# Aatricks/LightDiffusion-Next

Hardware: AMD Instinct MI355X
Metric: sampler it/s (UNet steps/sec) SD1.5 1024x1024 bs=1 bf16 (higher is better)
Workload: dtype bf16

## Files before the change

### lightdiffusion-next_amd/csrc/ff_block.hip

```cpp
#include <hip/hip_runtime.h>
#include <stdint.h>
#include <stdlib.h>
#include "ldx_device.h"
#include "ldx_kernels.h"
#include "rowblock_store.h"

namespace ldx {

constexpr int FB_C = 320, FB_I = 1280, FB_BM = 128, FB_CH = 128, FB_NCH = FB_I / FB_CH;
constexpr int FB_AROW = FB_C * 2 + 16;
constexpr int FB_GROW = FB_CH * 2 + 16;
constexpr int FB_ABYTES = FB_BM * FB_AROW, FB_GBYTES = FB_BM * FB_GROW;
constexpr int FB_LDS = FB_ABYTES + 2 * FB_GBYTES + 2 * FB_C * 4;
static_assert(FB_C == RB_C && FB_BM == RB_BM && FB_AROW == RB_AROW, "rb_layernorm_rows writes this A tile");

template <typename T>
__global__ __launch_bounds__(512, 1) void ff_block_kernel(const FFBlockArgs p) {
    extern __shared__ __attribute__((aligned(16))) char smem[];
    using V8 = typename Vec<T>::v8;
    char* sA = smem;
    char* sGb = smem + FB_ABYTES;
    float* sG = (float*)(smem + FB_ABYTES + 2 * FB_GBYTES);
    float* sBt = sG + FB_C;
    const int tid = threadIdx.x, lane = tid & 63;
    const int wave = __builtin_amdgcn_readfirstlane(tid >> 6);
    const int l15 = lane & 15, g4 = lane >> 4;
    const long m0 = (long)blockIdx.x * FB_BM;
    T* __restrict__ Hp = (T*)p.H;
    const T* __restrict__ W1 = (const T*)p.W1;
    const T* __restrict__ W2 = (const T*)p.W2;

    for (int i = tid; i < FB_C; i += 512) { sG[i] = p.ln_g[i]; sBt[i] = p.ln_b[i]; }
    rb_layernorm_rows<T>(Hp, p.ldh, m0, p.M, p.eps, sG, sBt, sA, tid, false);
    __syncthreads();

    f32x4 y[3][8];
#pragma unroll
    for (int t = 0; t < 3; ++t)
#pragma unroll
        for (int qt = 0; qt < 8; ++qt) y[t][qt] = (f32x4){0.f, 0.f, 0.f, 0.f};

    constexpr int NKS = FB_C / 32, PD = 2;
    uint4 w1[PD + 1][2];
    auto w1_rows = [&](int ch, const T*& wv, const T*& wg) __attribute__((always_inline)) {
        const int i0 = ch * FB_CH + wave * 16;
        const int vrow = (i0 >> 5) * 64 + (i0 & 31) + l15;
        wv = W1 + (long)vrow * FB_C + g4 * 8;
        wg = wv + 32 * FB_C;
    };
    {
        const T *wv, *wg;
        w1_rows(0, wv, wg);
#pragma unroll
        for (int ks = 0; ks < PD; ++ks) { w1[ks][0] = *(const uint4*)(wv + ks * 32); w1[ks][1] = *(const uint4*)(wg + ks * 32); }
    }
    auto w2_load = [&](int ch, int ks, uint4 (&w2f)[4][3]) __attribute__((always_inline)) {
        const T* w2 = W2 + (long)(wave * 40) * FB_I + ch * FB_CH + g4 * 8;
#pragma unroll
        for (int t = 0; t < 3; ++t) {
            const int r = 16 * t + l15;
            w2f[ks][t] = (r < 40) ? *(const uint4*)(w2 + (long)r * FB_I + ks * 32) : make_uint4(0, 0, 0, 0);
        }
    };
    for (int ch = 0; ch < FB_NCH; ++ch) {
        char* sGc = sGb + (ch & 1) * FB_GBYTES;
        uint4 w2f[4][3];
        {
            const T *wv, *wg;
            w1_rows(ch, wv, wg);
            f32x4 tv[8], tg[8];
#pragma unroll
            for (int qt = 0; qt < 8; ++qt) { tv[qt] = (f32x4){0.f, 0.f, 0.f, 0.f}; tg[qt] = (f32x4){0.f, 0.f, 0.f, 0.f}; }
#pragma unroll
            for (int ks = 0; ks < NKS; ++ks) {
                if (ks + PD < NKS) { w1[(ks + PD) % (PD + 1)][0] = *(const uint4*)(wv + (ks + PD) * 32); w1[(ks + PD) % (PD + 1)][1] = *(const uint4*)(wg + (ks + PD) * 32); }
                V8 af[8];
#pragma unroll
                for (int qt = 0; qt < 8; ++qt) af[qt] = as_v8<T>(*(const uint4*)(sA + (16 * qt + l15) * FB_AROW + (ks * 32 + g4 * 8) * 2));
                const V8 a8 = as_v8<T>(w1[ks % (PD + 1)][0]), g8 = as_v8<T>(w1[ks % (PD + 1)][1]);
#pragma unroll
                for (int qt = 0; qt < 8; ++qt) { tv[qt] = mfma16(a8, af[qt], tv[qt]); tg[qt] = mfma16(g8, af[qt], tg[qt]); }
                __builtin_amdgcn_sched_barrier(0);
            }
            w2_load(ch, 0, w2f);
            const int i0 = ch * FB_CH + wave * 16;
            const int brow = (i0 >> 5) * 64 + (i0 & 31) + 4 * g4;
            const float4 bv = *(const float4*)(p.b1 + brow), bg = *(const float4*)(p.b1 + brow + 32);
#pragma unroll
            for (int qt = 0; qt < 8; ++qt) {
                const float v0 = (tv[qt][0] + bv.x) * gelu_erf_f(tg[qt][0] + bg.x), v1 = (tv[qt][1] + bv.y) * gelu_erf_f(tg[qt][1] + bg.y);
                const float v2 = (tv[qt][2] + bv.z) * gelu_erf_f(tg[qt][2] + bg.z), v3 = (tv[qt][3] + bv.w) * gelu_erf_f(tg[qt][3] + bg.w);
                *(uint2*)(sGc + (16 * qt + l15) * FB_GROW + (wave * 16 + 4 * g4) * 2) = pack4<T>(v0, v1, v2, v3);
            }
        }
        __syncthreads();
        w2_load(ch, 1, w2f); w2_load(ch, 2, w2f); w2_load(ch, 3, w2f);
        if (ch + 1 < FB_NCH) {
            const T *wv, *wg;
            w1_rows(ch + 1, wv, wg);
#pragma unroll
            for (int ks = 0; ks < PD; ++ks) { w1[ks][0] = *(const uint4*)(wv + ks * 32); w1[ks][1] = *(const uint4*)(wg + ks * 32); }
        }
#pragma unroll
        for (int ks = 0; ks < 4; ++ks) {
            V8 gf[8];
#pragma unroll
            for (int qt = 0; qt < 8; ++qt) gf[qt] = as_v8<T>(*(const uint4*)(sGc + (16 * qt + l15) * FB_GROW + (ks * 32 + g4 * 8) * 2));
#pragma unroll
            for (int t = 0; t < 3; ++t) {
                const V8 w8 = as_v8<T>(w2f[ks][t]);
#pragma unroll
                for (int qt = 0; qt < 8; ++qt) y[t][qt] = mfma16(w8, gf[qt], y[t][qt]);
            }
            __builtin_amdgcn_sched_barrier(0);
        }
    }

    uint2 rr[3][8];
#pragma unroll
    for (int t = 0; t < 3; ++t)
#pragma unroll
        for (int qt = 0; qt < 8; ++qt) {
            const long m = m0 + 16 * qt + l15;
            const int nl = 16 * t + 4 * g4;
            rr[t][qt] = (m < p.M && nl < 40) ? *(const uint2*)(Hp + m * p.ldh + wave * 40 + nl) : make_uint2(0u, 0u);
        }
#pragma unroll
    for (int t = 0; t < 3; ++t) {
        const int nl = 16 * t + 4 * g4;
        const int n = wave * 40 + (nl < 40 ? nl : 0);
        const float4 bo = p.b2 ? *(const float4*)(p.b2 + n) : make_float4(0.f, 0.f, 0.f, 0.f);
#pragma unroll
        for (int qt = 0; qt < 8; ++qt) {
            float r4[4];
            unpack4<T>(rr[t][qt], r4);
            rr[t][qt] = pack4<T>(y[t][qt][0] + bo.x + r4[0], y[t][qt][1] + bo.y + r4[1], y[t][qt][2] + bo.z + r4[2], y[t][qt][3] + bo.w + r4[3]);
        }
    }
    __syncthreads();
    rb_store_rows<T, 8>(Hp, p.ldh, m0, p.M, 0, wave, l15, g4, tid, rr, sGb);
}

bool ff_block_ok(const FFBlockArgs& a) {
    return g_plan_sw.ff_fuse && a.C == FB_C && a.inner == FB_I && a.M > 0 && a.ldh % 8 == 0 && a.b1 != nullptr;
}
template <typename T>
static void launch_ff_t(const FFBlockArgs& a, hipStream_t s) {
    static DevOnce once;
    set_dyn_lds(once, (const void*)ff_block_kernel<T>, FB_LDS);
    hipLaunchKernelGGL((ff_block_kernel<T>), dim3((unsigned)((a.M + FB_BM - 1) / FB_BM)), dim3(512), FB_LDS, s, a);
}
void launch_ff_block(const FFBlockArgs& a, DType dt, hipStream_t s) {
    if (dt == DT_BF16) launch_ff_t<__bf16>(a, s); else launch_ff_t<_Float16>(a, s);
}

}
```

### lightdiffusion-next_amd/csrc/rowblock_store.h

```cpp
#pragma once
#include "ldx_device.h"

namespace ldx {

constexpr int RB_SROW = 320 * 2 + 16;
constexpr int RB_STAGE_BYTES = 64 * RB_SROW;
constexpr int RB_C = 320, RB_BM = 128;
constexpr int RB_AROW = RB_C * 2 + 16;

template <typename T>
__device__ __forceinline__ void rb_layernorm_rows(const T* __restrict__ Hp, const int ldh, const long m0, const long M, const float eps, const float* sG,
                                                  const float* sBt, char* sA, const int tid, const bool no_loads) {
    const int row = tid >> 2, part = tid & 3;
    const long m = m0 + row;
    float x[80];
    if (m < M && !no_loads) {
#pragma unroll
        for (int j = 0; j < 10; ++j) {
            const uint4 u = *(const uint4*)(Hp + m * ldh + (part + 4 * j) * 8);
            float f[8];
            unpack8<T>(u, f);
#pragma unroll
            for (int e = 0; e < 8; ++e) x[8 * j + e] = f[e];
        }
    } else {
#pragma unroll
        for (int e = 0; e < 80; ++e) x[e] = 0.f;
    }
    float su = 0.f;
#pragma unroll
    for (int e = 0; e < 80; ++e) su += x[e];
    su += dpp_f<0xB1>(su); su += dpp_f<0x4E>(su);
    const float mean = su * (1.0f / RB_C);
    float sq = 0.f;
#pragma unroll
    for (int e = 0; e < 80; ++e) { const float d = x[e] - mean; sq = fmaf(d, d, sq); }
    sq += dpp_f<0xB1>(sq); sq += dpp_f<0x4E>(sq);
    const float rstd = rsqrtf(sq * (1.0f / RB_C) + eps);
    __syncthreads();
#pragma unroll
    for (int j = 0; j < 10; ++j) {
        const int c0 = (part + 4 * j) * 8;
        float f[8];
#pragma unroll
        for (int e = 0; e < 8; ++e) f[e] = fmaf((x[8 * j + e] - mean) * rstd, sG[c0 + e], sBt[c0 + e]);
        *(uint4*)(sA + row * RB_AROW + c0 * 2) = pack8<T>(f);
    }
}

template <typename T, int QT>
__device__ __forceinline__ void rb_store_rows(T* __restrict__ Y, const int ldy, const long m0, const long M, const int col0, const int wave, const int l15,
                                              const int g4, const int tid, const uint2 (&out)[3][QT], char* sS, const long dup_rows = 0) {
    int tid_ = tid, l15_ = l15;
    asm volatile("" : "+v"(tid_), "+v"(l15_));
#pragma unroll
    for (int hh = 0; hh < QT / 4; ++hh) {
#pragma unroll
        for (int t = 0; t < 3; ++t) {
            const int nl = 16 * t + 4 * g4;
            if (nl < 40) {
#pragma unroll
                for (int q4 = 0; q4 < 4; ++q4) *(uint2*)(sS + (16 * q4 + l15_) * RB_SROW + (wave * 40 + nl) * 2) = out[t][4 * hh + q4];
            }
        }
        __syncthreads();
#pragma unroll
        for (int j = 0; j < 5; ++j) {
            const int idx = tid_ + 512 * j, row = idx / 40, ch = idx - row * 40;
            const long m = m0 + 64 * hh + row;
            if (m < M) {
                const uint4 v = *(const uint4*)(sS + row * RB_SROW + ch * 16);
                *(uint4*)(Y + m * ldy + col0 + ch * 8) = v;
                if (dup_rows) *(uint4*)(Y + (m + dup_rows) * ldy + col0 + ch * 8) = v;
            }
        }
        __syncthreads();
    }
}

}
```

### lightdiffusion-next_amd/csrc/rowgemm.hip

```cpp
#include <hip/hip_runtime.h>
#include <stdint.h>
#include <stdlib.h>
#include "ldx_device.h"
#include "ldx_kernels.h"
#include "rowblock_store.h"

namespace ldx {

template <int CC> struct RgGeom {
    static constexpr int BM = 128 * 320 / CC, QT = BM / 16, LPR = 512 / BM, NH = CC / 320;
    static constexpr int AROW = CC * 2 + 16, ABYTES = BM * AROW;
    static constexpr int TAB = 2 * CC * 4 + 8 * 64 * 4 + 64 * 4;
    static constexpr int LDS = ABYTES + TAB + RB_STAGE_BYTES;
};

template <typename T, int PRO, int CC>
__global__ __launch_bounds__(512, 1) void rowgemm_kernel(const RowGemmArgs p) {
    using G = RgGeom<CC>;
    constexpr int RG_C = CC, RG_BM = G::BM, RG_AROW = G::AROW, RG_ABYTES = G::ABYTES, QT = G::QT, LPR = G::LPR;
    extern __shared__ __attribute__((aligned(16))) char smem[];
    using V8 = typename Vec<T>::v8;
    char* sA = smem;
    float* sSc = (float*)(smem + RG_ABYTES);
    float* sSh = sSc + RG_C;
    float* sRed = sSh + RG_C;
    float* sMR = sRed + 8 * 64;
    const int tid = threadIdx.x, lane = tid & 63;
    const int wave = __builtin_amdgcn_readfirstlane(tid >> 6);
    const int l15_0 = lane & 15, g4_0 = lane >> 4;
    const long m0 = (long)blockIdx.x * RG_BM;
    const T* __restrict__ Xp = (const T*)p.X;
    const T* __restrict__ W = (const T*)p.W;

    const int nown = p.N / G::NH;
    const int npass = nown / 320;
    constexpr int NKS = RG_C / 32, PD = 3;
    uint4 wf[PD + 1][3];
    auto wload = [&](int wrow0_, int l15_, int g4_, int ks, int slot) __attribute__((always_inline)) {
#pragma unroll
        for (int t = 0; t < 3; ++t) {
            const int r = 16 * t + l15_;
            wf[slot][t] = (r < 40) ? *(const uint4*)(W + (long)(wrow0_ + r) * RG_C + ks * 32 + g4_ * 8) : make_uint4(0, 0, 0, 0);
        }
    };
#pragma unroll
    for (int ks = 0; ks < PD; ++ks) wload((int)blockIdx.y * nown + wave * 40, l15_0, g4_0, ks, ks);

    if (PRO == 1) { for (int i = tid; i < RG_C; i += 512) { sSc[i] = p.g[i]; sSh[i] = p.b[i]; } }
    if (PRO == 2) {
        const int b = (int)(m0 / p.HW);
        const int g = tid & 31, st = (tid >> 5) & 1, sl = tid >> 6;
        float a = 0.f;
        {
            const float* pp = p.partial + ((long)b * p.nchunk) * p.G * 2 + g * 2 + st;
            int ck = sl;
            for (; ck + 56 < p.nchunk; ck += 64) {
                float v[8];
#pragma unroll
                for (int u = 0; u < 8; ++u) v[u] = pp[(long)(ck + 8 * u) * p.G * 2];
#pragma unroll
                for (int u = 0; u < 8; ++u) a += v[u];
            }
            for (; ck < p.nchunk; ck += 8) a += pp[(long)ck * p.G * 2];
        }
        sRed[sl * 64 + g * 2 + st] = a;
        __syncthreads();
        if (tid < 32) {
            float su = 0.f, sq = 0.f;
#pragma unroll
            for (int s8 = 0; s8 < 8; ++s8) { su += sRed[s8 * 64 + tid * 2]; sq += sRed[s8 * 64 + tid * 2 + 1]; }
            const float n = (float)p.HW * (float)(RG_C / 32);
            const float mean = su / n;
            const float var = fmaxf(sq / n - mean * mean, 0.f);
            sMR[tid] = mean; sMR[32 + tid] = rsqrtf(var + p.eps);
        }
        __syncthreads();
        for (int c = tid; c < RG_C; c += 512) {
            const int g2 = c / (RG_C / 32);
            const float a2 = sMR[32 + g2] * p.g[c];
            sSc[c] = a2; sSh[c] = p.b[c] - sMR[g2] * a2;
        }
    }
    {
        const int row = tid / LPR, part = tid % LPR;
        const long m = m0 + row;
        uint4 raw[10];
#pragma unroll
        for (int j = 0; j < 10; ++j) raw[j] = (m < p.M && !(p.abl & 4)) ? *(const uint4*)(Xp + m * p.ldx + (part + LPR * j) * 8) : make_uint4(0, 0, 0, 0);
        if (PRO == 0) {
#pragma unroll
            for (int j = 0; j < 10; ++j) *(uint4*)(sA + row * RG_AROW + (part + LPR * j) * 16) = raw[j];
        } else {
            float x[80];
#pragma unroll
            for (int j = 0; j < 10; ++j) {
                float f[8];
                unpack8<T>(raw[j], f);
#pragma unroll
                for (int e = 0; e < 8; ++e) x[8 * j + e] = f[e];
            }
            float mean = 0.f, rstd = 1.f;
            if (PRO == 1) {
                float su = 0.f;
#pragma unroll
                for (int e = 0; e < 80; ++e) su += x[e];
                su += dpp_f<0xB1>(su); su += dpp_f<0x4E>(su); if (LPR == 8) su += dpp_f<0x141>(su);
                mean = su * (1.0f / RG_C);
                float sq = 0.f;
#pragma unroll
                for (int e = 0; e < 80; ++e) { const float d = x[e] - mean; sq = fmaf(d, d, sq); }
                sq += dpp_f<0xB1>(sq); sq += dpp_f<0x4E>(sq); if (LPR == 8) sq += dpp_f<0x141>(sq);
                rstd = rsqrtf(sq * (1.0f / RG_C) + p.eps);
            }
            __syncthreads();
#pragma unroll
            for (int j = 0; j < 10; ++j) {
                const int c0 = (part + LPR * j) * 8;
                float f[8];
#pragma unroll
                for (int e = 0; e < 8; ++e)
                    f[e] = (PRO == 1) ? fmaf((x[8 * j + e] - mean) * rstd, sSc[c0 + e], sSh[c0 + e]) : fmaf(x[8 * j + e], sSc[c0 + e], sSh[c0 + e]);
                *(uint4*)(sA + row * RG_AROW + c0 * 2) = pack8<T>(f);
            }
        }
    }
    __syncthreads();

#pragma unroll 1
    for (int pass = 0; pass < npass; ++pass) {
        int l15 = l15_0, g4 = g4_0;
        asm volatile("" : "+v"(l15), "+v"(g4));
        const int wrow0 = (int)blockIdx.y * nown + pass * 320 + wave * 40;
        f32x4 acc[3][QT];
#pragma unroll
        for (int t = 0; t < 3; ++t)
#pragma unroll
            for (int qt = 0; qt < QT; ++qt) acc[t][qt] = (f32x4){0.f, 0.f, 0.f, 0.f};
        if (!(p.abl & 2))
#pragma unroll
        for (int ks = 0; ks < NKS; ++ks) {
            if (ks + PD < NKS) wload(wrow0, l15, g4, ks + PD, (ks + PD) % (PD + 1));
            V8 af[QT];
#pragma unroll
            for (int qt = 0; qt < QT; ++qt) af[qt] = as_v8<T>(*(const uint4*)(sA + (16 * qt + l15) * RG_AROW + (ks * 32 + g4 * 8) * 2));
#pragma unroll
            for (int t = 0; t < 3; ++t) {
                const V8 w8 = as_v8<T>(wf[ks % (PD + 1)][t]);
#pragma unroll
                for (int qt = 0; qt < QT; ++qt) acc[t][qt] = mfma16(w8, af[qt], acc[t][qt]);
            }
            __builtin_amdgcn_sched_barrier(0);
        }
        __builtin_amdgcn_sched_barrier(0);
        uint2 rr[3][QT];
#pragma unroll
        for (int t = 0; t < 3; ++t)
#pragma unroll
            for (int qt = 0; qt < QT; ++qt) {
                const long m = m0 + 16 * qt + l15;
                const int nl = 16 * t + 4 * g4;
                rr[t][qt] = (p.R && m < p.M && nl < 40 && !(p.abl & 1)) ? *(const uint2*)((const T*)p.R + m * p.ldr + wrow0 + nl) : make_uint2(0u, 0u);
            }
#pragma unroll
        for (int t = 0; t < 3; ++t) {
            const int nl = 16 * t + 4 * g4;
            const int n = wrow0 + (nl < 40 ? nl : 0);
            const float4 bo = p.bias ? *(const float4*)(p.bias + n) : make_float4(0.f, 0.f, 0.f, 0.f);
#pragma unroll
            for (int qt = 0; qt < QT; ++qt) {
                float r4[4];
                unpack4<T>(rr[t][qt], r4);
                rr[t][qt] = pack4<T>(acc[t][qt][0] + bo.x + r4[0], acc[t][qt][1] + bo.y + r4[1], acc[t][qt][2] + bo.z + r4[2], acc[t][qt][3] + bo.w + r4[3]);
            }
        }
        if (p.gn_out) {
            float cs[3][4], cq[3][4];
#pragma unroll
            for (int t = 0; t < 3; ++t) {
#pragma unroll
                for (int r = 0; r < 4; ++r) { cs[t][r] = 0.f; cq[t][r] = 0.f; }
#pragma unroll
                for (int qt = 0; qt < QT; ++qt) {
                    float v4[4];
                    unpack4<T>(rr[t][qt], v4);
#pragma unroll
                    for (int r = 0; r < 4; ++r) { cs[t][r] += v4[r]; cq[t][r] = fmaf(v4[r], v4[r], cq[t][r]); }
                }
#pragma unroll
                for (int r = 0; r < 4; ++r) { cs[t][r] = row16_sum(cs[t][r]); cq[t][r] = row16_sum(cq[t][r]); }
                const int nl = 16 * t + 4 * g4;
                if (l15 == 0 && nl < 40) {
#pragma unroll
                    for (int r = 0; r < 4; ++r) { sSc[(wave * 40 + nl + r) * 2] = cs[t][r]; sSc[(wave * 40 + nl + r) * 2 + 1] = cq[t][r]; }
                }
            }
            __syncthreads();
            const int cpg = p.N / 32;
            if (tid < (320 / cpg) * 2) {
                const int gl = tid >> 1, st = tid & 1;
                float a = 0.f;
                for (int c = 0; c < cpg; ++c) a += sSc[(gl * cpg + c) * 2 + st];
                const int bimg = (int)(m0 / p.HW), chunk = (int)((m0 - (long)bimg * p.HW) / RG_BM);
                const int g0 = ((int)blockIdx.y * nown + pass * 320) / cpg;
                p.gn_out[(((long)bimg * p.gn_nchunk + chunk) * 32 + g0 + gl) * 2 + st] = a;
            }
        }
        if (pass + 1 < npass) {
#pragma unroll
            for (int ks = 0; ks < PD; ++ks) wload(wrow0 + 320, l15, g4, ks, ks);
        }
        if (!(p.abl & 8)) rb_store_rows<T, QT>((T*)p.Y, p.ldy, m0, p.M, (int)blockIdx.y * nown + pass * 320, wave, l15, g4, tid, rr, smem + RG_ABYTES + G::TAB, p.dup_rows);
    }
}

bool rowgemm_ok(const RowGemmArgs& a) {
    if (!g_plan_sw.rowgemm || (a.K != 320 && a.K != 640) || (a.K == 640 && !g_plan_sw.rowgemm640) || a.N <= 0 || a.N % a.K || a.M <= 0 || a.ldx % 8 || a.ldy % 8 || (a.R && a.ldr % 4) || a.pro < 0 || a.pro > 2) return false;
    const int bm = 128 * 320 / a.K;
    if (a.pro >= 1 && (!a.g || !a.b)) return false;
    if (a.pro == 2 && (!a.partial || a.G != 32 || a.HW % bm || a.M % a.HW || a.nchunk < 1 || a.nchunk > GN_NCHUNK)) return false;
    return true;
}
template <typename T, int PRO, int CC>
static void launch_rowgemm_inst(const RowGemmArgs& a, hipStream_t s) {
    using G = RgGeom<CC>;
    static DevOnce once;
    set_dyn_lds(once, (const void*)rowgemm_kernel<T, PRO, CC>, G::LDS);
    hipLaunchKernelGGL((rowgemm_kernel<T, PRO, CC>), dim3((unsigned)((a.M + G::BM - 1) / G::BM), G::NH), dim3(512), G::LDS, s, a);
}
template <typename T>
static void launch_rowgemm_t(const RowGemmArgs& a, hipStream_t s) {
    if (a.K == 320) {
        if (a.pro == 0) launch_rowgemm_inst<T, 0, 320>(a, s); else if (a.pro == 1) launch_rowgemm_inst<T, 1, 320>(a, s); else launch_rowgemm_inst<T, 2, 320>(a, s);
    } else {
        if (a.pro == 0) launch_rowgemm_inst<T, 0, 640>(a, s); else if (a.pro == 1) launch_rowgemm_inst<T, 1, 640>(a, s); else launch_rowgemm_inst<T, 2, 640>(a, s);
    }
}
void launch_rowgemm(const RowGemmArgs& a0, DType dt, hipStream_t s) {
    static const int abl = getenv("LDX_RG_ABL") ? atoi(getenv("LDX_RG_ABL")) : 0;
    RowGemmArgs a = a0; a.abl = abl;
    if (dt == DT_BF16) launch_rowgemm_t<__bf16>(a, s); else launch_rowgemm_t<_Float16>(a, s);
}

}
```

### lightdiffusion-next_amd/csrc/xattn_block.hip

```cpp
#include <hip/hip_runtime.h>
#include <stdint.h>
#include <stdlib.h>
#include "ldx_device.h"
#include "ldx_kernels.h"
#include "rowblock_store.h"

namespace ldx {

#ifdef XA_ABLATE
__device__ int xa_dbg = 0;
#define XA_DBG(bit) (xa_dbg & (bit))
#else
#define XA_DBG(bit) false
#endif
constexpr int XA_C = 320, XA_H = 8, XA_D = 40, XA_BM = 128, XA_MK = 80;
constexpr int XA_AROW = XA_C * 2 + 16;
constexpr int XA_VROW = 96;
constexpr int XA_ABYTES = XA_BM * XA_AROW, XA_VBYTES = XA_MK * XA_VROW;
constexpr int XA_LDS = XA_ABYTES + XA_H * XA_VBYTES + 2 * XA_C * 4;
static_assert(XA_C == RB_C && XA_BM == RB_BM && XA_AROW == RB_AROW, "rb_layernorm_rows writes this A tile");

template <typename T>
__device__ __forceinline__ void xa_project(const T* __restrict__ W, const int wrow0, const char* sA, const int l15, const int g4, f32x4 (&acc)[3][8]) {
    using V8 = typename Vec<T>::v8;
    constexpr int NKS = XA_C / 32, PD = 3;
#pragma unroll
    for (int t = 0; t < 3; ++t)
#pragma unroll
        for (int qt = 0; qt < 8; ++qt) acc[t][qt] = (f32x4){0.f, 0.f, 0.f, 0.f};
    uint4 wf[PD + 1][3];
    auto wload = [&](int ks, int slot) __attribute__((always_inline)) {
#pragma unroll
        for (int t = 0; t < 3; ++t) {
            const int r = 16 * t + l15;
            uint4 u = make_uint4(0, 0, 0, 0);
            if (r < XA_D) u = *(const uint4*)(W + (long)(wrow0 + r) * XA_C + ks * 32 + g4 * 8);
            wf[slot][t] = u;
        }
    };
#pragma unroll
    for (int ks = 0; ks < PD; ++ks) wload(ks, ks);
#pragma unroll
    for (int ks = 0; ks < NKS; ++ks) {
        if (ks + PD < NKS) wload(ks + PD, (ks + PD) % (PD + 1));
        V8 af[8];
#pragma unroll
        for (int qt = 0; qt < 8; ++qt) af[qt] = as_v8<T>(*(const uint4*)(sA + (16 * qt + l15) * XA_AROW + (ks * 32 + g4 * 8) * 2));
#pragma unroll
        for (int t = 0; t < 3; ++t) {
            const V8 w8 = as_v8<T>(wf[ks % (PD + 1)][t]);
#pragma unroll
            for (int qt = 0; qt < 8; ++qt) acc[t][qt] = mfma16(w8, af[qt], acc[t][qt]);
        }
    }
}

template <typename T>
__global__ __launch_bounds__(512, 1) void xattn_block_kernel(const XAttnArgs p) {
    extern __shared__ __attribute__((aligned(16))) char smem[];
    using V8 = typename Vec<T>::v8;
    char* sA = smem;
    float* sG = (float*)(smem + XA_ABYTES + XA_H * XA_VBYTES);
    float* sBt = sG + XA_C;
    const int tid = threadIdx.x, lane = tid & 63;
    const int wave = __builtin_amdgcn_readfirstlane(tid >> 6);
    const int l15 = lane & 15, g4 = lane >> 4;
    char* sV = smem + XA_ABYTES + wave * XA_VBYTES;
    const long m0 = (long)blockIdx.x * XA_BM;
    const int b = (int)(m0 / p.N);
    T* __restrict__ Hp = (T*)p.H;

    for (int i = tid; i < XA_C; i += 512) { sG[i] = p.ln_g[i]; sBt[i] = p.ln_b[i]; }
    {
        const T* __restrict__ Vp = (const T*)p.V + (long)b * p.Mk * p.ldv + wave * XA_D;
        for (int i = lane; i < XA_VBYTES / 16; i += 64) {
            const int row = i / 6, ch = i - row * 6;
            uint4 u = make_uint4(0, 0, 0, 0);
            if (row < p.Mk && ch < 5) u = *(const uint4*)(Vp + (long)row * p.ldv + ch * 8);
            *(uint4*)(sV + row * XA_VROW + ch * 16) = u;
        }
    }
    rb_layernorm_rows<T>(Hp, p.ldh, m0, p.M, p.eps, sG, sBt, sA, tid, XA_DBG(16));
    __syncthreads();

    f32x4 qT[3][8];
    if (!XA_DBG(1)) xa_project<T>((const T*)p.Wq, wave * XA_D, sA, l15, g4, qT);
    else for (int t = 0; t < 3; ++t) for (int qt = 0; qt < 8; ++qt) qT[t][qt] = (f32x4){1.f, 1.f, 1.f, 1.f};

    V8 kf[5][2];
    {
        const T* __restrict__ Kp = (const T*)p.K + (long)b * p.Mk * p.ldk + wave * XA_D;
#pragma unroll
        for (int kt = 0; kt < 5; ++kt) {
            const int key = 16 * kt + l15;
            uint2 a0 = make_uint2(0, 0), a1 = make_uint2(0, 0), a2 = make_uint2(0, 0);
            if (key < p.Mk) {
                const T* kr = Kp + (long)key * p.ldk;
                a0 = *(const uint2*)(kr + 4 * g4);
                a1 = *(const uint2*)(kr + 16 + 4 * g4);
                if (g4 < 2) a2 = *(const uint2*)(kr + 32 + 4 * g4);
            }
            kf[kt][0] = as_v8<T>(make_uint4(a0.x, a0.y, a1.x, a1.y));
            kf[kt][1] = as_v8<T>(make_uint4(a2.x, a2.y, 0u, 0u));
        }
    }
    V8 vf[3][3];
#pragma unroll
    for (int dt = 0; dt < 3; ++dt)
#pragma unroll
        for (int j = 0; j < 3; ++j) {
            const char* vp = sV + (j * 32 + g4 * 4 + (l15 >> 2)) * XA_VROW + (dt * 16 + (l15 & 3) * 4) * 2;
            U128 u;
            u.d[0] = lds_read_tr16(vp);
            u.d[1] = (j < 2) ? lds_read_tr16(vp + 16 * XA_VROW) : make_uint2(0u, 0u);
            vf[dt][j] = as_v8<T>(u.u);
        }
    __syncthreads();

    const float c = p.scale * 1.44269504088896340736f;
#pragma unroll
    for (int qt = 0; qt < 8; ++qt) {
        if (XA_DBG(2)) break;
        V8 qb0, qb1;
#pragma unroll
        for (int e = 0; e < 4; ++e) {
            qb0[e] = (T)qT[0][qt][e]; qb0[4 + e] = (T)qT[1][qt][e];
            qb1[e] = (g4 < 2) ? (T)qT[2][qt][e] : (T)0.f; qb1[4 + e] = (T)0.f;
        }
        f32x4 s[5];
#pragma unroll
        for (int kt = 0; kt < 5; ++kt) {
            s[kt] = mfma16(kf[kt][0], qb0, (f32x4){0.f, 0.f, 0.f, 0.f});
            s[kt] = mfma16(kf[kt][1], qb1, s[kt]);
        }
        float mx = -INFINITY;
#pragma unroll
        for (int kt = 0; kt < 5; ++kt)
#pragma unroll
            for (int r = 0; r < 4; ++r) {
                if (16 * kt + 4 * g4 + r >= p.Mk) s[kt][r] = -INFINITY;
                mx = fmaxf(mx, s[kt][r]);
            }
        mx = quad_max(mx);
        const float mc = (mx == -INFINITY) ? 0.f : mx * c;
        float pv[6][4], l = 0.f;
#pragma unroll
        for (int kt = 0; kt < 5; ++kt)
#pragma unroll
            for (int r = 0; r < 4; ++r) {
                const float e = to_f32(from_f32<T>(__builtin_amdgcn_exp2f(fmaf(s[kt][r], c, -mc))));
                pv[kt][r] = e; l += e;
            }
#pragma unroll
        for (int r = 0; r < 4; ++r) pv[5][r] = 0.f;
        l = quad_sum(l);
        f32x4 o[3];
#pragma unroll
        for (int dt = 0; dt < 3; ++dt) o[dt] = (f32x4){0.f, 0.f, 0.f, 0.f};
#pragma unroll
        for (int j = 0; j < 3; ++j) {
            V8 pf;
#pragma unroll
            for (int r = 0; r < 4; ++r) { pf[r] = (T)pv[2 * j][r]; pf[4 + r] = (T)pv[2 * j + 1][r]; }
#pragma unroll
            for (int dt = 0; dt < 3; ++dt) o[dt] = mfma16(vf[dt][j], pf, o[dt]);
        }
        const float inv = (l > 0.f) ? 1.0f / l : 0.f;
        const int q = 16 * qt + l15;
#pragma unroll
        for (int dt = 0; dt < 3; ++dt) {
            const int d = 16 * dt + 4 * g4;
            if (d < XA_D) *(uint2*)(sA + q * XA_AROW + (wave * XA_D + d) * 2) = pack4<T>(o[dt][0] * inv, o[dt][1] * inv, o[dt][2] * inv, o[dt][3] * inv);
        }
    }
    __syncthreads();

    f32x4 y[3][8];
    if (!XA_DBG(4)) xa_project<T>((const T*)p.Wo, wave * XA_D, sA, l15, g4, y);
    else for (int t = 0; t < 3; ++t) for (int qt = 0; qt < 8; ++qt) y[t][qt] = (f32x4){1.f, 1.f, 1.f, 1.f};
    if (XA_DBG(8)) return;
    uint2 rr[3][8];
#pragma unroll
    for (int t = 0; t < 3; ++t)
#pragma unroll
        for (int qt = 0; qt < 8; ++qt) {
            const long m = m0 + 16 * qt + l15;
            const int nl = 16 * t + 4 * g4;
            rr[t][qt] = (m < p.M && nl < XA_D && !XA_DBG(8)) ? *(const uint2*)(Hp + m * p.ldh + wave * XA_D + nl) : make_uint2(0u, 0u);
        }
#pragma unroll
    for (int t = 0; t < 3; ++t) {
        const int nl = 16 * t + 4 * g4;
        const int n = wave * XA_D + (nl < XA_D ? nl : 0);
        const float4 bo = p.bo ? *(const float4*)(p.bo + n) : make_float4(0.f, 0.f, 0.f, 0.f);
#pragma unroll
        for (int qt = 0; qt < 8; ++qt) {
            float r4[4];
            unpack4<T>(rr[t][qt], r4);
            rr[t][qt] = pack4<T>(y[t][qt][0] + bo.x + r4[0], y[t][qt][1] + bo.y + r4[1], y[t][qt][2] + bo.z + r4[2], y[t][qt][3] + bo.w + r4[3]);
        }
    }
    rb_store_rows<T, 8>(Hp, p.ldh, m0, p.M, 0, wave, l15, g4, tid, rr, smem + XA_ABYTES);
}

bool xattn_block_ok(const XAttnArgs& a) {
    return g_plan_sw.xattn_fuse && a.C == XA_C && a.heads == XA_H && a.Mk >= 1 && a.Mk <= XA_MK && a.N % XA_BM == 0 && a.M % a.N == 0 && a.ldh % 8 == 0 && a.ldk % 4 == 0 && a.ldv % 8 == 0;
}

template <typename T>
static void launch_xattn_t(const XAttnArgs& a, hipStream_t s) {
    static DevOnce once;
    set_dyn_lds(once, (const void*)xattn_block_kernel<T>, XA_LDS);
#ifdef XA_ABLATE
    static const int dbg_once = []() { const int v = getenv("LDX_XA_DBG") ? atoi(getenv("LDX_XA_DBG")) : 0; (void)hipMemcpyToSymbol(HIP_SYMBOL(xa_dbg), &v, sizeof(int)); return v; }();
    (void)dbg_once;
#endif
    hipLaunchKernelGGL((xattn_block_kernel<T>), dim3((unsigned)((a.M + XA_BM - 1) / XA_BM)), dim3(512), XA_LDS, s, a);
}
void launch_xattn_block(const XAttnArgs& a, DType dt, hipStream_t s) {
    if (dt == DT_BF16) launch_xattn_t<__bf16>(a, s); else launch_xattn_t<_Float16>(a, s);
}

}
```

Measured before the change: 76.62.

## Swizzle LDS operand tiles instead of padding to remove bank conflicts

Replaces the +16-byte row padding of the A, G and output staging tiles in LDS with an XOR swizzle of 16-byte chunks. This covers the ff, xattn and rowblock-store paths, and rowgemm's A stride becomes +32. A constexpr bank-conflict model checks at compile time that fragment reads are conflict-free and that stores are at most 2-way. The aim is to remove the 2-way conflicts the +16 stride caused on MFMA operand reads. In exchange it adds address arithmetic and an XOR-indexed layout that every writer and reader must follow consistently.

Measured after the change: 76.55. About the same (-0.1%).

```diff
diff --git a/lightdiffusion-next_amd/csrc/ff_block.hip b/lightdiffusion-next_amd/csrc/ff_block.hip
--- a/lightdiffusion-next_amd/csrc/ff_block.hip
+++ b/lightdiffusion-next_amd/csrc/ff_block.hip
@@ -8,11 +8,16 @@
 namespace ldx {
 
 constexpr int FB_C = 320, FB_I = 1280, FB_BM = 128, FB_CH = 128, FB_NCH = FB_I / FB_CH;
-constexpr int FB_AROW = FB_C * 2 + 16;
-constexpr int FB_GROW = FB_CH * 2 + 16;
+constexpr int FB_AROW = FB_C * 2;
+constexpr int FB_GROW = FB_CH * 2;
 constexpr int FB_ABYTES = FB_BM * FB_AROW, FB_GBYTES = FB_BM * FB_GROW;
-constexpr int FB_LDS = FB_ABYTES + 2 * FB_GBYTES + 2 * FB_C * 4;
+constexpr int FB_LDS_USED = FB_ABYTES + 2 * FB_GBYTES + 2 * FB_C * 4;
+constexpr int FB_LDS = FB_BM * (FB_C * 2 + 16) + 2 * FB_BM * (FB_CH * 2 + 16) + 2 * FB_C * 4;
 static_assert(FB_C == RB_C && FB_BM == RB_BM && FB_AROW == RB_AROW, "rb_layernorm_rows writes this A tile");
+static_assert(rb_opnd_read_cycles(FB_AROW, FB_C * 2) == lds::READ_B128.floor && rb_opnd_read_cycles(FB_GROW, FB_CH * 2) == lds::READ_B128.floor,
+              "fragment reads of A and G must be conflict-free");
+static_assert(rb_opnd_colstore_cycles(FB_GROW) <= 8, "GEGLU stores: 2-way at most (the floor for 16 rows x 8 bytes)");
+static_assert(FB_LDS_USED <= FB_LDS && FB_LDS <= lds::LDS_BYTES_PER_CU && RB_STAGE_BYTES <= 2 * FB_GBYTES, "LDS budget; the output tile goes over the G buffers");
 
 template <typename T>
 __global__ __launch_bounds__(512, 1) void ff_block_kernel(const FFBlockArgs p) {
@@ -25,6 +30,8 @@
     const int tid = threadIdx.x, lane = tid & 63;
     const int wave = __builtin_amdgcn_readfirstlane(tid >> 6);
     const int l15 = lane & 15, g4 = lane >> 4;
+    const RbFragLane a_lane = rb_frag_lane(l15, g4);
+    const int g_lane = rb_opnd_ofs(l15, g4, FB_GROW);
     const long m0 = (long)blockIdx.x * FB_BM;
     T* __restrict__ Hp = (T*)p.H;
     const T* __restrict__ W1 = (const T*)p.W1;
@@ -76,7 +83,7 @@
                 if (ks + PD < NKS) { w1[(ks + PD) % (PD + 1)][0] = *(const uint4*)(wv + (ks + PD) * 32); w1[(ks + PD) % (PD + 1)][1] = *(const uint4*)(wg + (ks + PD) * 32); }
                 V8 af[8];
 #pragma unroll
-                for (int qt = 0; qt < 8; ++qt) af[qt] = as_v8<T>(*(const uint4*)(sA + (16 * qt + l15) * FB_AROW + (ks * 32 + g4 * 8) * 2));
+                for (int qt = 0; qt < 8; ++qt) af[qt] = as_v8<T>(*(const uint4*)(sA + 16 * qt * FB_AROW + ks * 64 + a_lane.base[ks & 1]));
                 const V8 a8 = as_v8<T>(w1[ks % (PD + 1)][0]), g8 = as_v8<T>(w1[ks % (PD + 1)][1]);
 #pragma unroll
                 for (int qt = 0; qt < 8; ++qt) { tv[qt] = mfma16(a8, af[qt], tv[qt]); tg[qt] = mfma16(g8, af[qt], tg[qt]); }
@@ -90,7 +97,7 @@
             for (int qt = 0; qt < 8; ++qt) {
                 const float v0 = (tv[qt][0] + bv.x) * gelu_erf_f(tg[qt][0] + bg.x), v1 = (tv[qt][1] + bv.y) * gelu_erf_f(tg[qt][1] + bg.y);
                 const float v2 = (tv[qt][2] + bv.z) * gelu_erf_f(tg[qt][2] + bg.z), v3 = (tv[qt][3] + bv.w) * gelu_erf_f(tg[qt][3] + bg.w);
-                *(uint2*)(sGc + (16 * qt + l15) * FB_GROW + (wave * 16 + 4 * g4) * 2) = pack4<T>(v0, v1, v2, v3);
+                *(uint2*)(sGc + 16 * qt * FB_GROW + rb_opnd_ofs(l15, 2 * wave + (g4 >> 1), FB_GROW) + (g4 & 1) * 8) = pack4<T>(v0, v1, v2, v3);
             }
         }
         __syncthreads();
@@ -105,7 +112,7 @@
         for (int ks = 0; ks < 4; ++ks) {
             V8 gf[8];
 #pragma unroll
-            for (int qt = 0; qt < 8; ++qt) gf[qt] = as_v8<T>(*(const uint4*)(sGc + (16 * qt + l15) * FB_GROW + (ks * 32 + g4 * 8) * 2));
+            for (int qt = 0; qt < 8; ++qt) gf[qt] = as_v8<T>(*(const uint4*)(sGc + 16 * qt * FB_GROW + (g_lane ^ (ks * 64))));
 #pragma unroll
             for (int t = 0; t < 3; ++t) {
                 const V8 w8 = as_v8<T>(w2f[ks][t]);
diff --git a/lightdiffusion-next_amd/csrc/lds_image.h b/lightdiffusion-next_amd/csrc/lds_image.h
--- /dev/null
+++ b/lightdiffusion-next_amd/csrc/lds_image.h
@@ -0,0 +1,72 @@
+#pragma once
+
+namespace ldx {
+namespace lds {
+
+struct Instr {
+    int ngroups, glanes;
+    int banks;
+    int dwords;
+    int floor;
+    int xfer;
+    bool contiguous;
+};
+
+constexpr Instr READ_B128{4, 16, 64, 4, 4, 4, false};
+constexpr Instr READ_B64{2, 32, 64, 2, 2, 2, true};
+constexpr Instr READ_B64_TR_B16{2, 32, 64, 2, 2, 2, true};
+constexpr Instr WRITE_B64{4, 16, 32, 2, 4, 6, true};
+constexpr Instr WRITE_B128{8, 8, 32, 4, 8, 13, true};
+
+constexpr int B128_GROUP_LANE[2][16] = {{0, 1, 2, 3, 12, 13, 14, 15, 20, 21, 22, 23, 24, 25, 26, 27}, {4, 5, 6, 7, 8, 9, 10, 11, 16, 17, 18, 19, 28, 29, 30, 31}};
+
+constexpr int group_lane(const Instr& in, int g, int i) {
+    return in.contiguous ? g * in.glanes + i : 32 * (g >> 1) + B128_GROUP_LANE[g & 1][i];
+}
+
+template <typename F>
+constexpr int cycles(const Instr& in, F addr) {
+    int total = 0;
+    for (int g = 0; g < in.ngroups; ++g) {
+        long seen[64][32] = {};
+        int cnt[64] = {};
+        int worst = 0;
+        for (int i = 0; i < in.glanes; ++i) {
+            const long a = addr(group_lane(in, g, i));
+            if (a < 0) continue;
+            for (int d = 0; d < in.dwords; ++d) {
+                const long dw = a / 4 + d;
+                const int b = (int)(dw % in.banks);
+                bool dup = false;
+                for (int k = 0; k < cnt[b]; ++k) dup = dup || seen[b][k] == dw + 1;
+                if (!dup) { seen[b][cnt[b]] = dw + 1; ++cnt[b]; }
+                if (cnt[b] > worst) worst = cnt[b];
+            }
+        }
+        total += worst;
+    }
+    return total;
+}
+
+template <typename F>
+constexpr int cost(const Instr& in, F addr) {
+    const int c = cycles(in, addr);
+    return c > in.xfer ? c : in.xfer;
+}
+
+constexpr int frag16_read_cycles(int stride, int base = 0) {
+    return cycles(READ_B128, [=](int lane) { return (long)base + (long)(lane & 15) * stride + (lane >> 4) * 16; });
+}
+constexpr int frag32_read_cycles(int stride, int base = 0) {
+    return cycles(READ_B128, [=](int lane) { return (long)base + (long)(lane & 31) * stride + (lane >> 5) * 16; });
+}
+constexpr int frag16_read_worst(int stride, int row_bytes) {
+    int w = 0;
+    for (int ks = 0; ks * 64 < row_bytes; ++ks) { const int c = frag16_read_cycles(stride, ks * 64); w = c > w ? c : w; }
+    return w;
+}
+
+constexpr int LDS_BYTES_PER_CU = 160 * 1024;
+
+}
+}
diff --git a/lightdiffusion-next_amd/csrc/rowblock_store.h b/lightdiffusion-next_amd/csrc/rowblock_store.h
--- a/lightdiffusion-next_amd/csrc/rowblock_store.h
+++ b/lightdiffusion-next_amd/csrc/rowblock_store.h
@@ -1,12 +1,72 @@
 #pragma once
 #include "ldx_device.h"
+#include "lds_image.h"
 
 namespace ldx {
 
-constexpr int RB_SROW = 320 * 2 + 16;
+constexpr int RB_C = 320, RB_BM = 128;
+constexpr int RB_AROW = RB_C * 2;
+constexpr int rb_opnd_swz(int row, int row_bytes) { return (row & 3) | (((row ^ (row >> 2)) & 1) << 2) | (row_bytes == 256 ? (row & 1) << 3 : 0); }
+constexpr int rb_opnd_ofs(int row, int chunk, int row_bytes) { return row * row_bytes + ((chunk ^ rb_opnd_swz(row, row_bytes)) << 4); }
+struct RbFragLane { int base[2]; };
+__device__ __forceinline__ RbFragLane rb_frag_lane(int l15, int g4) {
+    const int f = rb_opnd_swz(l15, RB_AROW), lo = l15 * RB_AROW + ((g4 ^ (f & 3)) << 4), k = (f >> 2) << 6;
+    return {{lo + k, lo - k}};
+}
+constexpr int rb_opnd_read_cycles(int row_bytes, int data_bytes, bool swz = true) {
+    int w = 0;
+    for (int ks = 0; ks * 64 < data_bytes; ++ks) {
+        const int c = lds::cycles(lds::READ_B128, [=](int lane) { return swz ? rb_opnd_ofs(lane & 15, 4 * ks + (lane >> 4), row_bytes) : (lane & 15) * row_bytes + ks * 64 + (lane >> 4) * 16; });
+        w = c > w ? c : w;
+    }
+    return w;
+}
+constexpr int rb_opnd_colstore_cycles(int row_bytes) {
+    int w = 0;
+    for (int p0 = 0; p0 * 8 < row_bytes; p0 += 2) {
+        const int c = lds::cycles(lds::WRITE_B64, [=](int lane) { const int p = p0 + (lane >> 4); return p * 8 < row_bytes ? rb_opnd_ofs(lane & 15, p >> 1, row_bytes) + (p & 1) * 8 : -1; });
+        w = c > w ? c : w;
+    }
+    return w;
+}
+constexpr int rb_opnd_rowstore_cycles(int row_bytes) {
+    int w = 0;
+    for (int j = 0; j * 64 < row_bytes; ++j) {
+        const int c = lds::cycles(lds::WRITE_B128, [=](int lane) { return rb_opnd_ofs(lane >> 2, (lane & 3) + 4 * j, row_bytes); });
+        w = c > w ? c : w;
+    }
+    return w;
+}
+static_assert(rb_opnd_read_cycles(RB_AROW, RB_C * 2) == lds::READ_B128.floor, "A-tile fragment reads must be conflict-free");
+static_assert(rb_opnd_read_cycles(RB_C * 2 + 16, RB_C * 2, false) == 8, "the model must see the 2-way conflict of the + 16 stride");
+static_assert(rb_opnd_colstore_cycles(RB_AROW) <= 8, "8-byte column stores into the A tile: 2-way at most");
+static_assert(rb_opnd_rowstore_cycles(RB_AROW) == lds::WRITE_B128.floor, "the prologue's row stores must be conflict-free");
+
+constexpr int RB_SROW = 320 * 2;
 constexpr int RB_STAGE_BYTES = 64 * RB_SROW;
-constexpr int RB_C = 320, RB_BM = 128;
-constexpr int RB_AROW = RB_C * 2 + 16;
+constexpr int rb_stage_ofs(int row, int chunk) { return row * RB_SROW + ((chunk ^ (row & 7)) << 4); }
+constexpr int rb_stage_read_cycles() {
+    int w = 0;
+    for (int k = 0; k < 40; ++k) {
+        const int c = lds::cycles(lds::READ_B128, [=](int lane) { const int idx = 64 * k + lane; return rb_stage_ofs(idx / 40, idx % 40); });
+        w = c > w ? c : w;
+    }
+    return w;
+}
+constexpr int rb_stage_store_cycles() {
+    int w = 0;
+    for (int wave = 0; wave < 8; ++wave)
+        for (int t = 0; t < 3; ++t) {
+            const int c = lds::cycles(lds::WRITE_B64, [=](int lane) {
+                const int nl = 16 * t + 4 * (lane >> 4), col = (wave * 40 + nl) * 2;
+                return nl < 40 ? rb_stage_ofs(lane & 15, col >> 4) + (col & 8) : -1;
+            });
+            w = c > w ? c : w;
+        }
+    return w;
+}
+static_assert(rb_stage_read_cycles() == lds::READ_B128.floor, "staged tile: every wave's read-back must be conflict-free");
+static_assert(rb_stage_store_cycles() <= 8, "staged tile: 8-byte stores 2-way at most");
 
 template <typename T>
 __device__ __forceinline__ void rb_layernorm_rows(const T* __restrict__ Hp, const int ldh, const long m0, const long M, const float eps, const float* sG,
@@ -44,7 +104,7 @@
         float f[8];
 #pragma unroll
         for (int e = 0; e < 8; ++e) f[e] = fmaf((x[8 * j + e] - mean) * rstd, sG[c0 + e], sBt[c0 + e]);
-        *(uint4*)(sA + row * RB_AROW + c0 * 2) = pack8<T>(f);
+        *(uint4*)(sA + rb_opnd_ofs(row, part + 4 * j, RB_AROW)) = pack8<T>(f);
     }
 }
 
@@ -59,8 +119,9 @@
         for (int t = 0; t < 3; ++t) {
             const int nl = 16 * t + 4 * g4;
             if (nl < 40) {
+                const int col = (wave * 40 + nl) * 2;
 #pragma unroll
-                for (int q4 = 0; q4 < 4; ++q4) *(uint2*)(sS + (16 * q4 + l15_) * RB_SROW + (wave * 40 + nl) * 2) = out[t][4 * hh + q4];
+                for (int q4 = 0; q4 < 4; ++q4) *(uint2*)(sS + 16 * q4 * RB_SROW + rb_stage_ofs(l15_, col >> 4) + (col & 8)) = out[t][4 * hh + q4];
             }
         }
         __syncthreads();
@@ -69,7 +130,7 @@
             const int idx = tid_ + 512 * j, row = idx / 40, ch = idx - row * 40;
             const long m = m0 + 64 * hh + row;
             if (m < M) {
-                const uint4 v = *(const uint4*)(sS + row * RB_SROW + ch * 16);
+                const uint4 v = *(const uint4*)(sS + rb_stage_ofs(row, ch));
                 *(uint4*)(Y + m * ldy + col0 + ch * 8) = v;
                 if (dup_rows) *(uint4*)(Y + (m + dup_rows) * ldy + col0 + ch * 8) = v;
             }
diff --git a/lightdiffusion-next_amd/csrc/rowgemm.hip b/lightdiffusion-next_amd/csrc/rowgemm.hip
--- a/lightdiffusion-next_amd/csrc/rowgemm.hip
+++ b/lightdiffusion-next_amd/csrc/rowgemm.hip
@@ -9,10 +9,16 @@
 
 template <int CC> struct RgGeom {
     static constexpr int BM = 128 * 320 / CC, QT = BM / 16, LPR = 512 / BM, NH = CC / 320;
-    static constexpr int AROW = CC * 2 + 16, ABYTES = BM * AROW;
+    static constexpr int AROW = CC * 2 + 32, ABYTES = BM * AROW;
     static constexpr int TAB = 2 * CC * 4 + 8 * 64 * 4 + 64 * 4;
-    static constexpr int LDS = ABYTES + TAB + RB_STAGE_BYTES;
+    static constexpr int STAGE_OFS = ABYTES + 2 * CC * 4;
+    static constexpr int LDS_USED = STAGE_OFS + RB_STAGE_BYTES > ABYTES + TAB ? STAGE_OFS + RB_STAGE_BYTES : ABYTES + TAB;
+    static constexpr int LDS = BM * (CC * 2 + 16) + TAB + 64 * (320 * 2 + 16);
+    static_assert(rb_opnd_read_cycles(AROW, CC * 2, false) == lds::READ_B128.floor, "A-tile fragment reads must be conflict-free");
+    static_assert(LDS_USED <= LDS && LDS <= lds::LDS_BYTES_PER_CU, "LDS budget");
 };
+template struct RgGeom<320>;
+template struct RgGeom<640>;
 
 template <typename T, int PRO, int CC>
 __global__ __launch_bounds__(512, 1) void rowgemm_kernel(const RowGemmArgs p) {
@@ -209,7 +215,7 @@
 #pragma unroll
             for (int ks = 0; ks < PD; ++ks) wload(wrow0 + 320, l15, g4, ks, ks);
         }
-        if (!(p.abl & 8)) rb_store_rows<T, QT>((T*)p.Y, p.ldy, m0, p.M, (int)blockIdx.y * nown + pass * 320, wave, l15, g4, tid, rr, smem + RG_ABYTES + G::TAB, p.dup_rows);
+        if (!(p.abl & 8)) rb_store_rows<T, QT>((T*)p.Y, p.ldy, m0, p.M, (int)blockIdx.y * nown + pass * 320, wave, l15, g4, tid, rr, smem + G::STAGE_OFS, p.dup_rows);
     }
 }
 
diff --git a/lightdiffusion-next_amd/csrc/xattn_block.hip b/lightdiffusion-next_amd/csrc/xattn_block.hip
--- a/lightdiffusion-next_amd/csrc/xattn_block.hip
+++ b/lightdiffusion-next_amd/csrc/xattn_block.hip
@@ -14,16 +14,38 @@
 #define XA_DBG(bit) false
 #endif
 constexpr int XA_C = 320, XA_H = 8, XA_D = 40, XA_BM = 128, XA_MK = 80;
-constexpr int XA_AROW = XA_C * 2 + 16;
+constexpr int XA_AROW = XA_C * 2;
 constexpr int XA_VROW = 96;
 constexpr int XA_ABYTES = XA_BM * XA_AROW, XA_VBYTES = XA_MK * XA_VROW;
-constexpr int XA_LDS = XA_ABYTES + XA_H * XA_VBYTES + 2 * XA_C * 4;
+constexpr int XA_LDS_USED = XA_ABYTES + XA_H * XA_VBYTES + 2 * XA_C * 4;
+constexpr int XA_LDS = XA_BM * (XA_C * 2 + 16) + XA_H * XA_VBYTES + 2 * XA_C * 4;
 static_assert(XA_C == RB_C && XA_BM == RB_BM && XA_AROW == RB_AROW, "rb_layernorm_rows writes this A tile");
+static_assert(rb_opnd_read_cycles(XA_AROW, XA_C * 2) == lds::READ_B128.floor, "fragment reads of A (phase 1) and of the attention output (phase 3) must be conflict-free");
+static_assert(rb_opnd_colstore_cycles(XA_AROW) <= 8, "attention-output stores into A: 2-way at most (the floor for 16 rows x 8 bytes)");
+constexpr int xa_v_read_cycles() {
+    int w = 0;
+    for (int dt = 0; dt < 3; ++dt) {
+        const int c = lds::cycles(lds::READ_B64_TR_B16, [=](int lane) { return (4 * (lane >> 4) + ((lane & 15) >> 2)) * XA_VROW + (dt * 16 + (lane & 3) * 4) * 2; });
+        w = c > w ? c : w;
+    }
+    return w;
+}
+constexpr int xa_v_store_cycles() {
+    int w = 0;
+    for (int i0 = 0; i0 < XA_VBYTES / 16; i0 += 64) {
+        const int c = lds::cycles(lds::WRITE_B128, [=](int lane) { const int i = i0 + lane; return i < XA_VBYTES / 16 ? (i / 6) * XA_VROW + (i % 6) * 16 : -1; });
+        w = c > w ? c : w;
+    }
+    return w;
+}
+static_assert(xa_v_read_cycles() == lds::READ_B64_TR_B16.floor && xa_v_store_cycles() == lds::WRITE_B128.floor, "V_h region: conflict-free both ways");
+static_assert(XA_LDS_USED <= XA_LDS && XA_LDS <= lds::LDS_BYTES_PER_CU && RB_STAGE_BYTES <= XA_H * XA_VBYTES, "LDS budget; the output tile goes over the V regions");
 
 template <typename T>
 __device__ __forceinline__ void xa_project(const T* __restrict__ W, const int wrow0, const char* sA, const int l15, const int g4, f32x4 (&acc)[3][8]) {
     using V8 = typename Vec<T>::v8;
     constexpr int NKS = XA_C / 32, PD = 3;
+    const RbFragLane a_lane = rb_frag_lane(l15, g4);
 #pragma unroll
     for (int t = 0; t < 3; ++t)
 #pragma unroll
@@ -45,7 +67,7 @@
         if (ks + PD < NKS) wload(ks + PD, (ks + PD) % (PD + 1));
         V8 af[8];
 #pragma unroll
-        for (int qt = 0; qt < 8; ++qt) af[qt] = as_v8<T>(*(const uint4*)(sA + (16 * qt + l15) * XA_AROW + (ks * 32 + g4 * 8) * 2));
+        for (int qt = 0; qt < 8; ++qt) af[qt] = as_v8<T>(*(const uint4*)(sA + 16 * qt * XA_AROW + ks * 64 + a_lane.base[ks & 1]));
 #pragma unroll
         for (int t = 0; t < 3; ++t) {
             const V8 w8 = as_v8<T>(wf[ks % (PD + 1)][t]);
@@ -170,7 +192,8 @@
 #pragma unroll
         for (int dt = 0; dt < 3; ++dt) {
             const int d = 16 * dt + 4 * g4;
-            if (d < XA_D) *(uint2*)(sA + q * XA_AROW + (wave * XA_D + d) * 2) = pack4<T>(o[dt][0] * inv, o[dt][1] * inv, o[dt][2] * inv, o[dt][3] * inv);
+            const int col = (wave * XA_D + d) * 2;
+            if (d < XA_D) *(uint2*)(sA + rb_opnd_ofs(q, col >> 4, XA_AROW) + (col & 8)) = pack4<T>(o[dt][0] * inv, o[dt][1] * inv, o[dt][2] * inv, o[dt][3] * inv);
         }
     }
     __syncthreads();
```
